# constantinpape/torch-em

Hardware: AMD Instinct MI355X
Metric: voxels/sec fwd+bwd, UNet3d 1x128^3 bs=2 (higher is better)
Workload: dtype f32-class (forward convs on normalised activations: fp32 operands split into 2 fp16 terms = 22 mantissa bits, lo plane scaled by 2^12 with its own fp32 accumulator, 3 fp16 MFMAs per product; other forward convs 3 bf16 terms / 6 MFMAs; data-gradient convs 2 bf16 terms / 3 MFMAs (16-bit products); WEI

## Files before the change

### torch_em_amd/csrc/capi.hip

```cpp
#include "tem_common.h"
#include "conv_internal.h"
#include "tem_act.h"
#include <stdarg.h>
#include <string.h>

static thread_local char g_err[512] = "";

void tem_set_error(const char* fmt, ...) {
    va_list ap;
    va_start(ap, fmt);
    vsnprintf(g_err, sizeof(g_err), fmt, ap);
    va_end(ap);
}

extern "C" const char* tem_last_error(void) { return g_err; }

struct TemOption {
    const char* name;
    long long def;
};
static const TemOption g_opt_table[TEM_OPT_COUNT] = {
    {"wgrad_zs", 3},
    {"wgrad_zs_persist", 1},
    {"wgrad_sums", 1},
    {"wgrad_sums_min_mb", 128},
    {"fwd_persistent", -1},
    {"conv_fwd_variant", -1},
    {"conv1x1_stream", 1},
    {"fwd_ksplit_chunks", 0},
    {"wgrad_cus", 256},
    {"upsample_generic", 0},
    {"team_min_units", 0},
    {"zr_splitk", 1},
    {"zr_wide", 1},
    {"zr_tile_blocks", 1},
    {"dice_vox", 1},
    {"upsample2_ch8", 1},
    {"pool_vec8", 2},
    {"fp32_zr", 1},
};
static long long g_opt_val[TEM_OPT_COUNT];
static bool g_opt_set[TEM_OPT_COUNT];

long long tem_option(int id) {
    if (id < 0 || id >= TEM_OPT_COUNT) return 0;
    return __atomic_load_n(&g_opt_set[id], __ATOMIC_RELAXED) ? __atomic_load_n(&g_opt_val[id], __ATOMIC_RELAXED)
                                                            : g_opt_table[id].def;
}
static int opt_find(const char* name) {
    if (!name) return -1;
    for (int i = 0; i < TEM_OPT_COUNT; ++i)
        if (!strcmp(name, g_opt_table[i].name)) return i;
    return -1;
}
extern "C" int tem_set_option(const char* name, int64_t value) {
    const int id = opt_find(name);
    TEM_REQUIRE(id >= 0, "tem_set_option: unknown option '%s'", name ? name : "(null)");
    __atomic_store_n(&g_opt_val[id], (long long)value, __ATOMIC_RELAXED);
    __atomic_store_n(&g_opt_set[id], true, __ATOMIC_RELAXED);
    return TEM_OK;
}
extern "C" int tem_get_option(const char* name, int64_t* value) {
    const int id = opt_find(name);
    TEM_REQUIRE(id >= 0 && value, "tem_get_option: unknown option '%s'", name ? name : "(null)");
    *value = (int64_t)tem_option(id);
    return TEM_OK;
}
extern "C" int tem_version(void) { return 100; }

extern "C" int tem_device_cus(void) {
    int dev = 0;
    if (hipGetDevice(&dev) != hipSuccess) return TEM_ELAUNCH;
// ... 169 lines not shown
```

### torch_em_amd/csrc/conv_internal.h

```cpp
#pragma once
#include <hip/hip_runtime.h>
#include <stdint.h>
#include "../../include/tem_hip.h"
#include "tem_common.h"

struct TemConvCall {
    int stx = 0;
    int sty = 0;
    int64_t x_cs = 0, y_cs = 0;
    TemByproducts* bp = nullptr;
    const unsigned* in_amax = nullptr;
    const float* ref_coef = nullptr;
    unsigned* g_amax_out = nullptr;
    const unsigned* g_amax_in = nullptr;

    bool wants(unsigned bit) const {
        if (!bp || (bp->delivered & bit)) return false;
        return bit == TEM_BP_NORM_COEF ? bp->coef != nullptr : bit == TEM_BP_NORM_SUMS ? bp->sums_part != nullptr : bp->out_amax != nullptr;
    }
    void delivered(unsigned bit) const { if (bp) bp->delivered |= bit; }
    unsigned* take_output_amax() const {
        if (!wants(TEM_BP_OUT_AMAX)) return nullptr;
        delivered(TEM_BP_OUT_AMAX);
        return bp->out_amax;
    }
};

struct TemConvShape {
    int N, D, H, W, Cin, Cout, kd, kh, kw;
    int64_t V() const { return (int64_t)D * H * W; }
    int64_t NV() const { return (int64_t)N * D * H * W; }
    int key() const { return (kd == 3) * 4 + (kh == 3) * 2 + (kw == 3); }
};

inline bool tem_plane32_ok(const TemConvShape& sh, int64_t ld) { return (int64_t)sh.H * sh.W * 8 * 4 * ld < (1ll << 31); }
inline long long tem_team_min_units(int forced) {
    const long long minu = tem_option(TEM_OPT_TEAM_MIN_UNITS);
    return tem_option(TEM_OPT_CONV_FWD_VARIANT) == forced ? 1 : (minu > 0 ? minu : 2ll * tem_ncu());
}
struct TemPatchTiling {
    bool flat;
    int TZ, TY, TX, NR;
    int64_t per, nblk;
    int ks;
};
TemPatchTiling tem_fwd_patch_tiling(const TemConvShape& sh);
struct ZrGeom {
    int shape_ok, ok;
    int nZ, nY, nX;
    int64_t nunits;
};
struct PpGeom {
    int variant;
    int TZ, TY, TX, CT, WM;
    int nZ, nY, nX;
    int64_t nunits;
};

int tem_conv_fwd_mfma(const TemPatchTiling& t, int ks, const float* x, int64_t x_ld, const float* scale, const float* shift,
                      const float* w_packed, const float* bias, float* y, int64_t y_ld, const float* ref, int64_t ref_ld, void* ws,
                      const TemConvShape& sh, int act, hipStream_t s);

int64_t tem_conv_wgrad_mfma_ws(int N, int D, int H, int W, int Cin, int Cout, int kd, int kh, int kw);
int tem_conv_wgrad_mfma(const float* x, int64_t x_ld, const float* scale, const float* shift, const float* g,
                        int64_t g_ld, float* dw_tap_ci_co, float* db, void* ws, int64_t ws_bytes, int N, int D, int H,
                        int W, int Cin, int Cout, int kd, int kh, int kw, int sd_layout, hipStream_t s);

bool tem_conv_fwd_cin1(const TemConvCall& c, const float* x, int64_t x_ld, const float* scale, const float* shift, const float* w,
                       const float* bias, float* y, int64_t y_ld, const float* ref, int N, int D, int H, int W,
                       int Cin, int Cout, int kd, int kh, int kw, int act, float* stat, hipStream_t s);
int64_t tem_conv_fwd_cin1_stat_blocks(int D, int H, int W, int Cin, int Cout, int kd, int kh, int kw);
int64_t tem_conv_wgrad_cin1_ws(int Cout, int ntaps);
bool tem_conv_wgrad_cin1(const TemConvCall& c, const float* x, int64_t x_ld, const float* scale, const float* shift, const float* g,
                         int64_t g_ld, float* dw, float* db, void* ws, int N, int D, int H, int W, int Cin, int Cout,
                         int kd, int kh, int kw, int sd_layout, const float* gnx, int64_t gnx_ld, const float* gcoef,
                         hipStream_t s);
bool tem_conv_fwd_cout1(const TemConvCall& c, const float* x, int64_t x_ld, const float* scale, const float* shift, const float* w,
                        const float* bias, float* y, int64_t y_ld, const float* ref, int N, int D, int H, int W,
                        int Cin, int Cout, int kd, int kh, int kw, int act, hipStream_t s);
bool tem_conv1x1_proj(const TemConvCall& c, const float* x, int64_t x_ld, const float* scale, const float* w, const float* bias, float* y,
                      int64_t y_ld, const float* ref, int64_t NV, int Cin, int Cout, int act, hipStream_t s);
int64_t tem_conv1x1_proj_wgrad_ws(int Cin, int Cout);
bool tem_conv1x1_proj_wgrad(const TemConvCall& c, const float* x, int64_t x_ld, const float* scale, const float* g, int64_t g_ld, float* dw,
// ... 73 lines not shown
```

### torch_em_amd/csrc/conv_zr.hip

```cpp
#include "tem_common.h"
#include "conv_internal.h"
#include "conv_arith.h"
#include "conv_split.h"
#include "tem_act.h"
#include <type_traits>

#ifndef TEM_ZR_PRIO
#define TEM_ZR_PRIO 1
#endif
#ifndef TEM_ZR_R0
#define TEM_ZR_R0 2
#endif
#ifndef TEM_ZR_R0_16
#define TEM_ZR_R0_16 2
#endif
#ifndef TEM_ZR_R0_16S
#define TEM_ZR_R0_16S 2
#endif
#ifndef TEM_ZR_AD
#define TEM_ZR_AD 2
#endif
#ifndef TEM_ZR_ST_AUX
#define TEM_ZR_ST_AUX 2
#endif
#ifndef TEM_ZR_ST_AUX_KS
#define TEM_ZR_ST_AUX_KS 2
#endif
#ifndef TEM_ZR_X32_R0_M0
#define TEM_ZR_X32_R0_M0 6
#define TEM_ZR_X32_R0_M1 4
#define TEM_ZR_X32_R0_M2 6
#define TEM_ZR_X32_R0_M3 5
#endif
#ifndef TEM_ZR_KS_FILL
#define TEM_ZR_KS_FILL 4
#endif
#ifndef TEM_ZR_ABL
#define TEM_ZR_ABL 0
#endif
#ifdef TEM_ZR_TRACE
#ifndef TEM_ZR_TRACE_BLOCK
#define TEM_ZR_TRACE_BLOCK 0
#endif
__device__ unsigned long long tem_zr_trace_buf[2][64][12];
// ... 65 lines not shown
    float a = r, b = r;
    asm volatile("s_nop 1\n\tv_permlane16_swap_b32 %0, %1" : "+v"(a), "+v"(b));
    return a + b;
}
__device__ __forceinline__ float zr_xor32_sum(float r) {
    float a = r, b = r;
    asm volatile("s_nop 1\n\tv_permlane32_swap_b32 %0, %1" : "+v"(a), "+v"(b));
    return a + b;
}

template <int CTRL>
__device__ __forceinline__ float zr_dpp(float v) {
    return __builtin_bit_cast(float, __builtin_amdgcn_update_dpp(0, __builtin_bit_cast(int, v), CTRL, 0xf, 0xf, true));
}

__device__ __forceinline__ unsigned zr_mix_lo(unsigned h, float g0, float g1) {
    unsigned q;
    const float c = -F16_LO_SCALE;
    asm("v_fma_mixlo_f16 %0, %1, %2, %3 op_sel_hi:[1,0,0]" : "=v"(q) : "v"(h), "s"(c), "v"(g0));
    asm("v_fma_mixhi_f16 %0, %1, %2, %3 op_sel:[1,0,0] op_sel_hi:[1,0,0]" : "+v"(q) : "v"(h), "s"(c), "v"(g1));
    return q;
}

__device__ __forceinline__ unsigned zr_ssel_ltu(unsigned a, unsigned b, unsigned t, unsigned f) {
    unsigned r;
    asm volatile("s_cmp_lt_u32 %1, %2\n\ts_cselect_b32 %0, %3, %4" : "=s"(r) : "s"(a), "s"(b), "s"(t), "s"(f) : "scc");
    return r;
}

struct ZrUnit {
    int cot, n, z0, y0, x0, ksl;
};

template <int NS, bool F16, int MODE, bool KSPLIT = false, bool WIDE = false, typename T = float, bool X32 = false, bool XS = false>
__global__ __launch_bounds__(XS ? 256 : 512, XS ? 1 : 2) void k_conv_zr(
    const T* __restrict__ x, int64_t x_ld, const float* __restrict__ scale, const float* __restrict__ shift,
    const uint4* __restrict__ wp, const float* __restrict__ bias, std::conditional_t<KSPLIT, float, T>* __restrict__ y, int64_t y_ld,
    const T* __restrict__ ref, int64_t ref_ld, int N, int D, int H, int W, int Cin, int Cout, int act, int nZ,
    int nY, int nX, float* __restrict__ stat, int nunits, const unsigned* __restrict__ in_amax, int ks, int blk,
    unsigned* __restrict__ out_amax, int64_t x_cs, int64_t y_cs) {
    static_assert(!KSPLIT || MODE == 0, "split-K units write raw partial sums");
    constexpr bool AMAX = MODE == 2 || MODE == 3;
    float amx = 0.f;
    static_assert(!WIDE || NS == 2, "the wide one-term kernel uses the two LDS planes of the two-term layout");
    static_assert(!X32 || (NS == 2 && !F16 && !WIDE && sizeof(T) == 4), "exact fp32: two LDS planes of eight fp32 channels, fp32 tensors");
    static_assert(!XS || X32, "the one-team workgroup exists for the exact-fp32 arithmetic only");
    constexpr bool T16 = sizeof(T) == 2;
    using TOut = std::conditional_t<KSPLIT, float, T>;
    constexpr bool Y16 = sizeof(TOut) == 2;
    constexpr int XB = (int)sizeof(T), YB = (int)sizeof(TOut);
    static_assert(!T16 || WIDE, "16-bit storage: 32 input channels per phase");
    constexpr int CK = WIDE ? 2 * BCK : BCK;
    constexpr int TZ = 4, TY = 16, TX = 8;
    constexpr int HZ = TZ + 2, HY = TY + 2, HX = TX + 2;
    constexpr int HV = HZ * HY * HX;
    constexpr int PLB = HV * 32;
    constexpr int NIT = HZ * 3;
    constexpr int LPV = (WIDE && !T16) ? 8 : 4;
    constexpr int SPP = (WIDE && !T16) ? 6 : 3;
    constexpr int CPL = T16 ? 8 : 4;
    constexpr int RP = NIT / SPP;
    constexpr int R0 = X32 ? (MODE == 0 ? TEM_ZR_X32_R0_M0 : MODE == 1 ? TEM_ZR_X32_R0_M1 : MODE == 2 ? TEM_ZR_X32_R0_M2 : TEM_ZR_X32_R0_M3)
                       : (WIDE && !T16) ? ((MODE == 1 || MODE == 3) ? 1 : 2)
                       : T16 ? ((MODE == 1 || MODE == 3) ? TEM_ZR_R0_16S : TEM_ZR_R0_16)
                             : (TEM_ZR_R0 < HZ ? TEM_ZR_R0 : HZ);
    constexpr int FR = NS * 64;
    constexpr bool SC = F16 && NS == 2 && !WIDE;
    constexpr int ZSTEP = HY * HX * 32;
    static_assert(HY % 2 == 0, "the record-half swizzle (row parity) is the same in every halo plane");
    extern __shared__ __attribute__((aligned(16))) unsigned char zr_lds[];

    if (SC) __builtin_amdgcn_s_setreg(1 | (23 << 6) | (0 << 11), 1);
    const int tid = threadIdx.x, lane = tid & 63;
    const int wv = __builtin_amdgcn_readfirstlane(tid >> 6);
    const int team = wv >> 2, tw = wv & 3, tl = tid & 255;
    const int kh = lane >> 5, v = lane & 31;
    const int vu = (int)((0x73261540u >> (4 * (v >> 2))) & 7u) * 4 + (v & 3);
    const int py = vu >> 3, px = vu & 7;
    unsigned char* lds = zr_lds + team * (NS * PLB);

    const int G = (XS ? 1 : 2) * gridDim.x;
    const int slot = XS ? tem_xcd_remap(blockIdx.x, gridDim.x) : tem_xcd_remap(blockIdx.x, gridDim.x) * 2 + team;
    const int ncot = Cout >> 5;
    const int nch_all = Cin / CK;
    const int nch = KSPLIT ? nch_all / ks : nch_all;
    const int my_units = slot < nunits ? (nunits - slot + G - 1) / G : 0;
    const int P = ((nunits + G - 1) / G) * nch;

    auto decode = [&](int ui) {
        int u = slot + ui * G;
        ZrUnit t;
        t.ksl = 0;
        if (KSPLIT) { t.ksl = u % ks; u /= ks; }
        t.cot = u % ncot; u /= ncot;
        const int lx = blk & 15, ly = (blk >> 4) & 15, lz = blk >> 8;
        const int b = u & ((1 << (lx + ly + lz)) - 1);
        u >>= lx + ly + lz;
        const int bx = b & ((1 << lx) - 1), by = (b >> lx) & ((1 << ly) - 1), bz = b >> (lx + ly);
        const int mX = nX >> lx, mY = nY >> ly, mZ = nZ >> lz;
        t.x0 = (((u % mX) << lx) + bx) * TX; u /= mX;
        t.y0 = (((u % mY) << ly) + by) * TY; u /= mY;
        t.z0 = (((u % mZ) << lz) + bz) * TZ; u /= mZ;
        t.n = u;
        return t;
    };

    const int c4 = tl & (LPV - 1);
    unsigned poff[SPP];
    unsigned lwj[SPP];
#pragma unroll
    for (int j = 0; j < SPP; ++j) {
        const int q = min((tl + 256 * j) / LPV, HY * HX - 1);
        const int hy = q / HX, hx = q % HX;
        poff[j] = ((unsigned)(hy * W + hx) * (unsigned)x_ld + (unsigned)(c4 * CPL)) * (unsigned)XB;
        if (T16 || X32)
            lwj[j] = (unsigned)(q * 32) + (unsigned)((((c4 & 1) ^ (hy & 1)) << 4)) + (unsigned)((c4 >> 1) * PLB);
        else
            lwj[j] = (unsigned)(q * 32) + (unsigned)(((((c4 >> 1) & 1) ^ (hy & 1)) << 4) | ((c4 & 1) << 3)) + (unsigned)((c4 >> 2) * PLB);
    }
    const unsigned ctr_off_ = ((unsigned)(W + 1) * (unsigned)x_ld + (unsigned)(c4 * CPL)) * (unsigned)XB;
    unsigned pvo[X32 ? SPP : 1];
    unsigned yxu = (1u << SPP) - 1u;
    auto unit_offsets = [&](const ZrUnit& t) {
        if constexpr (X32) {
            yxu = 0;
#pragma unroll
            for (int j = 0; j < SPP; ++j) {
                const int q = min((tl + 256 * j) / LPV, HY * HX - 1);
                const unsigned gy = (unsigned)(t.y0 - 1 + q / HX), gx = (unsigned)(t.x0 - 1 + q % HX);
                const bool ok = (gy < (unsigned)H) & (gx < (unsigned)W);
                yxu |= ok ? (1u << j) : 0u;
                pvo[X32 ? j : 0] = ok ? poff[j] : ctr_off_;
            }
        }
    };
    const bool slot2 = tl < (HY * HX * LPV - 256 * (SPP - 1));
    const unsigned ctr_off = ((unsigned)(W + 1) * (unsigned)x_ld + (unsigned)(c4 * CPL)) * (unsigned)XB;
    const unsigned plane_b = (unsigned)(H * W) * (unsigned)x_ld * (unsigned)XB;
    const int hvb = (4 * tw + py) * HX + px;
    const unsigned yoff_lane = ((unsigned)(4 * tw * W + (lane >> 3)) * (unsigned)y_ld + (unsigned)(4 * (lane & 7))) * (unsigned)YB;
    const unsigned roff_lane = ((unsigned)(4 * tw * W + (lane >> 3)) * (unsigned)ref_ld + (unsigned)(4 * (lane & 7))) * (unsigned)XB;
    const __amdgpu_buffer_rsrc_t rw = zr_rsrc(wp);
    const unsigned woff_lane = (unsigned)lane * 16u;
    const float act_floor = act == TEM_ACT_RELU ? 0.f : -__builtin_inff();
    float psc = 1.f, pinv = 1.f;
    if (in_amax) {
        const int e = (int)((*in_amax >> 23) & 0xffu);
        const int k = e == 0 ? 0 : min(max(141 - e, -100), 100);
        psc = __builtin_bit_cast(float, (unsigned)(127 + k) << 23);
        pinv = __builtin_bit_cast(float, (unsigned)(127 - k) << 23);
    }

    floatx16 acc[TZ];
    floatx16 accl[SC ? TZ : 1];
    const int tapstride = nch_all * FR;

    int ui = 0, ci = 0;
    ZrUnit cu = decode(0), eu = cu;
    unit_offsets(cu);
    bool epi_pending = false;
    float bv = (bias && my_units > 0) ? bias[cu.cot * 32 + v] : 0.f;
    float bve = 0.f;
    auto bias16 = [&](float* b16, float bsrc) {
#pragma unroll
        for (int i = 0; i < 16; ++i) {
            const int c0 = 8 * (i >> 2) + (i & 3);
            const float lo = __builtin_bit_cast(float, __builtin_amdgcn_readlane(__builtin_bit_cast(int, bsrc), c0));
            const float hi = __builtin_bit_cast(float, __builtin_amdgcn_readlane(__builtin_bit_cast(int, bsrc), c0 + 4));
            b16[i] = kh ? hi : lo;
        }
    };
#pragma unroll
    for (int z = 0; z < TZ; ++z)
#pragma unroll
        for (int i = 0; i < 16; ++i) {
            acc[z][i] = 0.f;
            if (SC) accl[SC ? z : 0][i] = 0.f;
        }
    unsigned wsoff = 0;

    auto epilogue_now = [&](unsigned yoff_l, unsigned roff_l, int s) {
        (void)s;
        if constexpr (X32) {
            int lane_ = (int)(threadIdx.x & 63);
            asm volatile("" : "+v"(lane_));
            const int lane = lane_, kh = lane >> 5, v = lane & 31;
            const int vu = (int)((0x73261540u >> (4 * (v >> 2))) & 7u) * 4 + (v & 3);
            const int py = vu >> 3, px = vu & 7;
            (void)py; (void)px; (void)kh;
#include "conv_zr_epilogue.inc"
        }
// ... 120 lines not shown
#pragma unroll
                    for (int pp = 0; pp < 2; ++pp) wqn[tz][pp] = zr_load4u(rw, woff_lane, wsoff_n + (unsigned)((tz * 9) * ts + pp * 64) * 16u);
                }
                stage_conv(u, tnxt);
#pragma unroll
                for (int c = 0; c < 4; ++c)
#pragma unroll
                    for (int tz = 0; tz < 3; ++tz)
#pragma unroll
                        for (int z = 0; z < TZ; ++z)
                            acc[z] = __builtin_amdgcn_mfma_f32_32x32x2f32(comp(wq[g & 1][tz][p], c), comp(xr[u & 1][z + tz], c), acc[z], 0, 0, 0);
                __builtin_amdgcn_sched_barrier(0);
            }
            if (last_chunk) {
                eu = cu;
                bve = bv;
                unsigned yo = yoff_lane, ro = roff_lane;
                asm volatile("" : "+v"(yo), "+v"(ro));
                epilogue_now(yo, ro, ph);
                bv = bias ? bias[tu.cot * 32 + v] : 0.f;
                ++ui;
            }
            cu = tu;
            ci = tc;
#pragma unroll
            for (int tz = 0; tz < 3; ++tz)
#pragma unroll
                for (int p = 0; p < 2; ++p) wq[0][tz][p] = wqn[tz][p];
            __syncthreads();
        }
        if (AMAX && out_amax) tem_amax_commit(out_amax, amx);
        return;
    }
    if (team) __syncthreads();
    for (int s = 0; s <= P; ++s) {
        const bool do_stage = ui < my_units;
        uint4 wq[2][3][NS];
        {
            ZR_STAMP(0);
#pragma unroll
            for (int j = 0; j < SPP; ++j) asm volatile("" : "+v"(lwj[j]), "+v"(poff[j]));
            unsigned yoff_l = yoff_lane, roff_l = roff_lane;
            asm volatile("" : "+v"(yoff_l), "+v"(roff_l));
            float4 tmp[NIT];
            unsigned inb[2] = {0xffffffffu, 0xffffffffu};
            float4 sc4 = make_float4(1.f, 1.f, 1.f, 1.f), sf4 = make_float4(0.f, 0.f, 0.f, 0.f);
            float4 sc5 = sc4, sf5 = sf4;
            bool interior = true;
            __amdgpu_buffer_rsrc_t rx = zr_rsrc(x);
            auto load_norm = [&]() {
                if (scale) {
                    sc4 = *reinterpret_cast<const float4*>(scale + (int64_t)cu.n * Cin + (cu.ksl * nch + ci) * CK + c4 * CPL);
                    sf4 = *reinterpret_cast<const float4*>(shift + (int64_t)cu.n * Cin + (cu.ksl * nch + ci) * CK + c4 * CPL);
                    if (T16) {
                        sc5 = *reinterpret_cast<const float4*>(scale + (int64_t)cu.n * Cin + (cu.ksl * nch + ci) * CK + c4 * CPL + 4);
                        sf5 = *reinterpret_cast<const float4*>(shift + (int64_t)cu.n * Cin + (cu.ksl * nch + ci) * CK + c4 * CPL + 4);
                    }
                } else if (in_amax) {
                    sc4 = make_float4(psc, psc, psc, psc);
                }
            };
            if (do_stage) {
                if constexpr (!X32) load_norm();
                const int64_t xch = (T16 && x_cs) ? (int64_t)(cu.ksl * nch + ci) * x_cs : (int64_t)((cu.ksl * nch + ci) * CK);
                const T* xb = x + ((((int64_t)cu.n * D + (cu.z0 - 1)) * H + (cu.y0 - 1)) * W + (cu.x0 - 1)) * x_ld + xch;
                rx = zr_rsrc((TEM_ZR_ABL & 64) ? x + xch : xb);
                interior = (cu.z0 >= 1) & (cu.z0 + HZ - 1 <= D) & (cu.y0 >= 1) & (cu.y0 + HY - 1 <= H) & (cu.x0 >= 1) &
                           (cu.x0 + HX - 1 <= W);
                if (TEM_ZR_ABL & 32) interior = true;
                if constexpr (X32) {
#pragma unroll
                    for (int hz = 0; hz < R0; ++hz) {
                        const unsigned so = zr_ssel_ltu((unsigned)(cu.z0 - 1 + hz), (unsigned)D, (unsigned)hz * plane_b, plane_b);
#pragma unroll
                        for (int j = 0; j < SPP; ++j) {
                            if (TEM_ZR_ABL & 1) tmp[hz * SPP + j] = make_float4(0.5f + hz, 0.25f, -1.f, 2.f);
                            else tmp[hz * SPP + j] = zr_load4(rx, pvo[X32 ? j : 0], so);
                        }
                    }
                    load_norm();
                }
            }
            unsigned yx = (1u << SPP) - 1u;
            if constexpr (X32) {
                if (do_stage) {
                    yx = yxu;
                    if (!interior) {
                        inb[0] = inb[1] = 0;
#pragma unroll
                        for (int hz = 0; hz < HZ; ++hz) {
                            const bool zok = (unsigned)(cu.z0 - 1 + hz) < (unsigned)D;
#pragma unroll
                            for (int j = 0; j < SPP; ++j)
                                inb[hz / 3] |= (zok & ((yx >> j) & 1u)) ? (1u << ((hz % 3) * SPP + j)) : 0u;
                        }
                    }
                }
            } else
            if (do_stage && !interior) {
                int tl_ = tl;
                asm volatile("" : "+v"(tl_));
                yx = 0;
#pragma unroll
                for (int j = 0; j < SPP; ++j) {
                    const int q = min((tl_ + 256 * j) / LPV, HY * HX - 1);
                    const unsigned gy = (unsigned)(cu.y0 - 1 + q / HX), gx = (unsigned)(cu.x0 - 1 + q % HX);
                    yx |= ((gy < (unsigned)H) & (gx < (unsigned)W)) ? (1u << j) : 0u;
                }
            }
            auto issue_loads = [&](auto interior_tag, auto lo_tag, auto hi_tag) {
                constexpr bool INTERIOR = decltype(interior_tag)::value;
                constexpr int LO = decltype(lo_tag)::value, HI = decltype(hi_tag)::value;
                if (INTERIOR) {
#pragma unroll
                    for (int hz = LO; hz < HI; ++hz)
#pragma unroll
                        for (int j = 0; j < SPP; ++j) {
                            if (TEM_ZR_ABL & 1) tmp[(hz % RP) * SPP + j] = make_float4(0.5f + hz, 0.25f, -1.f, 2.f);
                            else tmp[(hz % RP) * SPP + j] = zr_load4(rx, poff[j], (unsigned)hz * plane_b);
                        }
                } else {
                    if (LO == 0) inb[0] = inb[1] = 0;
#pragma unroll
                    for (int hz = LO; hz < HI; ++hz) {
                        const bool zok = (unsigned)(cu.z0 - 1 + hz) < (unsigned)D;
#pragma unroll
                        for (int j = 0; j < SPP; ++j) {
                            const bool ok = zok & ((yx >> j) & 1u);
                            inb[hz / 3] |= ok ? (1u << ((hz % 3) * SPP + j)) : 0u;
                            tmp[(hz % RP) * SPP + j] = zr_load4(rx, (ok ? poff[j] : ctr_off) + (ok ? (unsigned)hz * plane_b : plane_b), 0);
                        }
                    }
                }
            };
            if (do_stage && !X32) {
                if (interior) issue_loads(std::true_type{}, std::integral_constant<int, 0>{}, std::integral_constant<int, R0>{});
                else issue_loads(std::false_type{}, std::integral_constant<int, 0>{}, std::integral_constant<int, R0>{});
            }
            ZR_STAMP(1);
            if (!X32 && epi_pending) {
#include "conv_zr_epilogue.inc"
                epi_pending = false;
                ZR_STAMP(11);
            }
            ZR_STAMP(6);
            if (do_stage) {
                auto convert = [&](auto interior_tag, auto hz_tag) {
                    constexpr bool INTERIOR = decltype(interior_tag)::value;
                    constexpr int hz = decltype(hz_tag)::value;
#pragma unroll
                    for (int j = 0; j < SPP; ++j) {
                        const int it = (hz % RP) * SPP + j;
                        if constexpr (T16) {
                            if (j < SPP - 1 || slot2) {
                                u32x4z raw = __builtin_bit_cast(u32x4z, floatx4z{tmp[it].x, tmp[it].y, tmp[it].z, tmp[it].w});
                                if (scale) {
                                    raw.x = zr_norm2<F16>(raw.x, sc4.x, sf4.x, sc4.y, sf4.y);
                                    raw.y = zr_norm2<F16>(raw.y, sc4.z, sf4.z, sc4.w, sf4.w);
                                    raw.z = zr_norm2<F16>(raw.z, sc5.x, sf5.x, sc5.y, sf5.y);
                                    raw.w = zr_norm2<F16>(raw.w, sc5.z, sf5.z, sc5.w, sf5.w);
                                }
                                if (!INTERIOR) {
                                    const bool ok = ((inb[hz / 3] >> ((hz % 3) * SPP + j)) & 1u) != 0;
                                    raw.x = ok ? raw.x : 0u; raw.y = ok ? raw.y : 0u; raw.z = ok ? raw.z : 0u; raw.w = ok ? raw.w : 0u;
                                }
                                if (!(TEM_ZR_ABL & 8) || raw.x == 0x12345678u)
                                    *reinterpret_cast<uint4*>(lds + lwj[j] + hz * ZSTEP) = make_uint4(raw.x, raw.y, raw.z, raw.w);
                            }
                        } else
                        if (j < SPP - 1 || slot2) {
                            float m = 1.f;
                            if (!INTERIOR) m = ((inb[hz / 3] >> ((hz % 3) * SPP + j)) & 1u) ? 1.f : 0.f;
                            float e[4] = {fmaf(tmp[it].x, sc4.x, sf4.x), fmaf(tmp[it].y, sc4.y, sf4.y),
                                          fmaf(tmp[it].z, sc4.z, sf4.z), fmaf(tmp[it].w, sc4.w, sf4.w)};
                            if (!INTERIOR) {
#pragma unroll
                                for (int c = 0; c < 4; ++c) e[c] *= m;
                            }
                            unsigned char* dstp = lds + lwj[j] + hz * ZSTEP;
                            if constexpr (X32) {
                                if (!(TEM_ZR_ABL & 8) || e[0] == 12345.678f) *reinterpret_cast<float4*>(dstp) = make_float4(e[0], e[1], e[2], e[3]);
                            } else
                            if (SC) {
                                const half2_t hh0 = {(_Float16)e[0], (_Float16)e[1]}, hh1 = {(_Float16)e[2], (_Float16)e[3]};
                                unsigned u0 = __builtin_bit_cast(unsigned, hh0), u1 = __builtin_bit_cast(unsigned, hh1);
                                if (!(TEM_ZR_ABL & 8) || u0 == 0x12345678u) *reinterpret_cast<uint2*>(dstp) = make_uint2(u0, u1);
                                const float g[4] = {e[0] * F16_LO_SCALE, e[1] * F16_LO_SCALE, e[2] * F16_LO_SCALE, e[3] * F16_LO_SCALE};
                                const unsigned q0 = zr_mix_lo(u0, g[0], g[1]), q1 = zr_mix_lo(u1, g[2], g[3]);
                                if (!(TEM_ZR_ABL & 8) || u0 == 0x12345678u) *reinterpret_cast<uint2*>(dstp + PLB) = make_uint2(q0, q1);
                            } else if (WIDE) {
#pragma unroll
                                for (int c = 0; c < 4; ++c) asm volatile("" : "+v"(e[c]));
                                const unsigned h0 = pk16<F16>(e[0], e[1]), h1 = pk16<F16>(e[2], e[3]);
                                if (!(TEM_ZR_ABL & 8) || h0 == 0x12345678u) *reinterpret_cast<uint2*>(dstp) = make_uint2(h0, h1);
                            } else {
                                if (F16 && NS == 1) {
#pragma unroll
                                    for (int c = 0; c < 4; ++c) asm volatile("" : "+v"(e[c]));
                                }
#pragma unroll
                                for (int p = 0; p < NS; ++p) {
                                    const unsigned h0 = pk16<F16>(e[0], e[1]), h1 = pk16<F16>(e[2], e[3]);
                                    if (!(TEM_ZR_ABL & 8) || h0 == 0x12345678u)
                                        *reinterpret_cast<uint2*>(dstp + p * PLB) = make_uint2(h0, h1);
                                    if (p + 1 < NS) {
                                        e[0] -= lo16<F16>(h0);
                                        e[1] -= hi16<F16>(h0);
                                        e[2] -= lo16<F16>(h1);
                                        e[3] -= hi16<F16>(h1);
                                    }
                                }
                            }
                        }
                    }
                };
                auto stage_planes = [&](auto interior_tag) {
#define ZR_PLANE(HZI)                                                                                              \
    do {                                                                                                           \
        if ((HZI) + R0 < HZ)                                                                                       \
            issue_loads(interior_tag, std::integral_constant<int, ((HZI) + R0 < HZ ? (HZI) + R0 : 0)>{},           \
                        std::integral_constant<int, ((HZI) + R0 < HZ ? (HZI) + R0 + 1 : 0)>{});                    \
        convert(interior_tag, std::integral_constant<int, (HZI)>{});                                               \
    } while (0)
                    ZR_PLANE(0); ZR_PLANE(1); ZR_PLANE(2); ZR_PLANE(3); ZR_PLANE(4); ZR_PLANE(5);
#undef ZR_PLANE
                };
                if (interior) stage_planes(std::true_type{});
                else stage_planes(std::false_type{});
                ZR_STAMP(7);
                wsoff = (unsigned)((cu.cot * 27 * nch_all + cu.ksl * nch + ci) * FR) * 16u;
#pragma unroll
                for (int tz = 0; tz < 3; ++tz)
#pragma unroll
                    for (int p = 0; p < NS; ++p)
                        wq[0][tz][p] = zr_load4u(rw, woff_lane, wsoff + (unsigned)((tz * 9) * tapstride + p * 64) * 16u);
            }
            ZR_STAMP(2);
        }
        __syncthreads();
        {
            ZR_STAMP(3);
            if (do_stage) {
                int ts = tapstride;
                asm volatile("" : "+s"(ts));
                if (TEM_ZR_PRIO) __builtin_amdgcn_s_setprio(TEM_ZR_PRIO);
                constexpr int NSTEP = 9 * HZ;
                constexpr int AD = TEM_ZR_AD;
                uint4 af[AD + 1][NS];
                unsigned a0 = 0u;
                const unsigned hsel = (unsigned)((py & 1) ^ kh) << 4;
                int hvb_ = hvb;
                asm volatile("" : "+v"(hvb_));
                auto col_addr = [&](int g) {
                    const int hvv = hvb_ + (g / 3) * HX + (g % 3);
                    a0 = (unsigned)hvv * 32u + (((g / 3) & 1) ? hsel ^ 16u : hsel);
                };
                auto a_read = [&](int st) {
                    const int hz = st % HZ;
#pragma unroll
                    for (int p = 0; p < NS; ++p)
                        af[st % (AD + 1)][p] = *reinterpret_cast<const uint4*>(lds + a0 + hz * ZSTEP + p * PLB);
                };
                if constexpr (X32) {
                    uint4 xr[2][HZ];
                    auto r_read = [&](int u) {
                        if ((u & 1) == 0) col_addr(u >> 1);
#pragma unroll
                        for (int hz = 0; hz < HZ; ++hz)
                            xr[u & 1][hz] = *reinterpret_cast<const uint4*>(lds + a0 + hz * ZSTEP + (u & 1) * PLB);
                    };
                    auto comp = [](const uint4& q, int c) {
                        return __builtin_bit_cast(float, c == 0 ? q.x : (c == 1 ? q.y : (c == 2 ? q.z : q.w)));
                    };
                    r_read(0);
#pragma unroll
// ... 45 lines not shown
#pragma unroll
                        for (int p = 0; p < 2; ++p)
#pragma unroll
                            for (int tz = 0; tz < 3; ++tz) {
                                const int z = hz - tz;
                                if (z < 0 || z >= TZ) continue;
                                acc[z] = mfma16<F16>(wq[g & 1][tz][p], a[p], acc[z]);
                            }
                    } else
#pragma unroll
                    for (int sum = NS - 1; sum >= 0; --sum)
#pragma unroll
                        for (int i = 0; i <= sum; ++i)
#pragma unroll
                            for (int tz = 0; tz < 3; ++tz) {
                                const int z = hz - tz;
                                if (z < 0 || z >= TZ) continue;
                                if (TEM_ZR_ABL & 16) {
                                    asm volatile("" ::"v"(a[sum - i].x), "v"(a[sum - i].w), "v"(wq[g & 1][tz][i].x), "v"(wq[g & 1][tz][i].w));
                                    continue;
                                }
                                if (SC && sum == 1)
                                    accl[SC ? z : 0] = mfma16<F16>(wq[g & 1][tz][i], a[sum - i], accl[SC ? z : 0]);
                                else
                                    acc[z] = mfma16<F16>(wq[g & 1][tz][i], a[sum - i], acc[z]);
                            }
                    __builtin_amdgcn_sched_barrier(0);
                }
                }
                if (TEM_ZR_PRIO) __builtin_amdgcn_s_setprio(0);
            }
            ZR_STAMP(4);
        }
        if (do_stage) {
            if (++ci == nch) {
                ci = 0;
                eu = cu;
                epi_pending = !X32;
                bve = bv;
                if constexpr (X32) {
                    unsigned yo = yoff_lane, ro = roff_lane;
                    asm volatile("" : "+v"(yo), "+v"(ro));
                    epilogue_now(yo, ro, s);
                }
                bv = 0.f;
                if (++ui < my_units) {
                    cu = decode(ui);
                    if (bias) bv = bias[cu.cot * 32 + v];
                    unit_offsets(cu);
                }
            }
        }
        __syncthreads();
        ZR_STAMP(5);
    }
    if (!team) __syncthreads();
    if (AMAX && out_amax) tem_amax_commit(out_amax, amx);
}

ZrGeom tem_zr_geometry(const TemConvCall& c, const TemConvShape& sh, int mode) {
    ZrGeom g = {};
    const long long opt = tem_option(TEM_OPT_CONV_FWD_VARIANT);
    if (opt == 0 || opt == 1) return g;
    if (!tem_zr_takes(mode, c, sh.Cin)) return g;
    if (sh.key() != 7 || sh.D < 4 || sh.Cin % 16 || sh.Cout % 32) return g;
    g.shape_ok = 1;
    g.nZ = (sh.D + 3) / 4;
    g.nY = (sh.H + 15) / 16;
    g.nX = (sh.W + 7) / 8;
    g.nunits = (int64_t)sh.N * g.nZ * g.nY * g.nX * (sh.Cout / 32);
    g.ok = g.nunits < (1ll << 31) && g.nunits >= tem_team_min_units(2);
    return g;
}

static int zr_tile_blocks(const ZrGeom& g) {
    if (!tem_option(TEM_OPT_ZR_TILE_BLOCKS)) return 0;
    auto lg = [](int n) { return n % 4 == 0 ? 2 : (n % 2 == 0 ? 1 : 0); };
    return lg(g.nX) | (lg(g.nY) << 4) | (lg(g.nZ) << 8);
}

template <int NS, bool F16, int MODE, bool KSPLIT = false, bool WIDE = false, typename T = float, bool X32 = false, bool XS = false>
static void zr_launch(const TemConvCall& c, const ZrGeom& g, const float* x_, int64_t x_ld, const float* scale, const float* shift, const float* wp,
                      const float* bias, float* y_, int64_t y_ld, const float* ref_, int64_t ref_ld, const TemConvShape& sh,
                      int act, float* stat, const unsigned* in_amax, hipStream_t s, int ks = 1) {
    constexpr size_t ldsb = (size_t)2 * NS * 1080 * 32 + 4 * 32 * 144;
    static_assert(ldsb <= 160 * 1024, "LDS budget");
    const T* x = reinterpret_cast<const T*>(x_);
    const T* ref = reinterpret_cast<const T*>(ref_);
    auto* y = reinterpret_cast<std::conditional_t<KSPLIT, float, T>*>(y_);
    auto kern = &k_conv_zr<NS, F16, MODE, KSPLIT, WIDE, T, X32, XS>;
    static bool attr = false;
    if (!attr) {
        (void)hipFuncSetAttribute(reinterpret_cast<const void*>(kern), hipFuncAttributeMaxDynamicSharedMemorySize, (int)ldsb);
        attr = true;
    }
    const int64_t nunits = g.nunits * ks;
    int64_t grid = XS ? nunits : (nunits + 1) / 2;
    if (grid > tem_ncu()) grid = tem_ncu();
    unsigned* const out_amax = (MODE == 2 || MODE == 3) ? c.take_output_amax() : nullptr;
    hipLaunchKernelGGL(kern, dim3((unsigned)grid), dim3(XS ? 256 : 512), ldsb, s, x, x_ld, scale, shift, reinterpret_cast<const uint4*>(wp),
                       bias, y, y_ld, ref, ref_ld, sh.N, sh.D, sh.H, sh.W, sh.Cin, sh.Cout, act, g.nZ, g.nY, g.nX, stat, (int)nunits, in_amax, ks,
                       zr_tile_blocks(g), out_amax, (int64_t)(sizeof(T) == 2 ? c.x_cs : 0), (int64_t)(sizeof(T) == 2 && !KSPLIT ? c.y_cs : 0));
}

template <int NS_, bool F16_, bool WIDE_ = false, typename T_ = float, bool X32_ = false, bool XS_ = false>
struct ZrVariant {
    static constexpr int NS = NS_;
    static constexpr bool F16 = F16_, WIDE = WIDE_, X32 = X32_, XS = XS_;
    using T = T_;
};
template <typename F>
static void zr_variant(const TemConvCall& c, int mode, bool wide, F&& f) {
    const TemArith& a = tem_arith(mode);
    if (c.stx == TEM_ST_F16) f(ZrVariant<2, true, true, tem_f16>{});
    else if (c.stx == TEM_ST_BF16) f(ZrVariant<2, false, true, tem_bf16>{});
    else if (mode == TEM_ARITH_FP32 && tem_option(TEM_OPT_FP32_ZR) == 2) f(ZrVariant<2, false, false, float, true, true>{});
    else if (mode == TEM_ARITH_FP32) f(ZrVariant<2, false, false, float, true>{});
    else if (a.planes == 1 && wide) tem_select_bool(a.elem == TEM_EL_F16, [&](auto f16) { f(ZrVariant<2, f16(), true>{}); });
    else if (a.planes == 1) tem_select_bool(a.elem == TEM_EL_F16, [&](auto f16) { f(ZrVariant<1, f16()>{}); });
    else tem_select_bool(a.pack == TEM_PK_F16_LO12, [&](auto f16) { f(ZrVariant<2, f16()>{}); });
}

int tem_zr_splitk_ks(const TemConvCall& c, const ZrGeom& g, const TemConvShape& sh, int mode) {
// ... 55 lines not shown
```

### torch_em_amd/csrc/tem_common.h

```cpp
#pragma once
#include <hip/hip_runtime.h>
#include <stdint.h>
#include <stdio.h>
#include "../../include/tem_hip.h"

void tem_set_error(const char* fmt, ...);

enum {
    TEM_OPT_WGRAD_ZS = 0,
    TEM_OPT_WGRAD_ZS_PERSIST,
    TEM_OPT_WGRAD_SUMS,
    TEM_OPT_WGRAD_SUMS_MIN_MB,
    TEM_OPT_FWD_PERSISTENT,
    TEM_OPT_CONV_FWD_VARIANT,
    TEM_OPT_CONV1X1_STREAM,
    TEM_OPT_FWD_KSPLIT_CHUNKS,
    TEM_OPT_WGRAD_CUS,
    TEM_OPT_UPSAMPLE_GENERIC,
    TEM_OPT_TEAM_MIN_UNITS,
    TEM_OPT_ZR_SPLITK,
    TEM_OPT_ZR_WIDE,
    TEM_OPT_ZR_TILE_BLOCKS,
    TEM_OPT_DICE_VOX,
    TEM_OPT_UPSAMPLE2_CH8,
    TEM_OPT_POOL_VEC8,
    TEM_OPT_FP32_ZR,
    TEM_OPT_COUNT
};
long long tem_option(int id);
int tem_ncu();

#define TEM_REQUIRE(cond, ...)                 \
    do {                                       \
        if (!(cond)) {                         \
            tem_set_error(__VA_ARGS__);        \
            return TEM_EINVAL;                 \
        }                                      \
    } while (0)

#define TEM_TRY(call)                          \
    do {                                       \
        const int rc__ = (call);               \
        if (rc__ != TEM_OK) return rc__;       \
    } while (0)

#define TEM_CHECK_LAUNCH(name)                                                   \
    do {                                                                         \
        hipError_t e__ = hipGetLastError();                                      \
        if (e__ != hipSuccess) {                                                 \
            tem_set_error("%s: launch failed: %s", name, hipGetErrorString(e__)); \
            return TEM_ELAUNCH;                                                  \
        }                                                                        \
    } while (0)

static inline int64_t tem_cdiv(int64_t a, int64_t b) { return (a + b - 1) / b; }
static inline int64_t tem_align_up(int64_t a, int64_t b) { return tem_cdiv(a, b) * b; }

static inline int tem_grid_1d(int64_t work_items, int block, int max_blocks = 256 * 8) {
    int64_t g = tem_cdiv(work_items, block);
// ... 37 lines not shown
```

Before: 275.6 million.

## Pair sibling teams to co-stage halves of one halo tile in shared LDS buffers

Adds a PAIR variant of the zero-redundancy forward conv kernel. The two teams in a workgroup each stage half of the z-halo planes of the same tile into a shared, double-buffered LDS region, and one team lags a step behind so that staging and MFMA tap work overlap. Unit decode is reordered so sibling slots share an input tile across output-channel tiles, and the pipeline runs one extra iteration with a conditional barrier. The aim is to halve per-team global loads and LDS staging. In exchange the sibling teams are now coupled, which adds synchronisation and some complexity in the barrier logic. It is enabled by default for fp32 two-plane modes when Cout is a multiple of 64.

```diff
diff --git a/torch_em_amd/csrc/capi.hip b/torch_em_amd/csrc/capi.hip
--- a/torch_em_amd/csrc/capi.hip
+++ b/torch_em_amd/csrc/capi.hip
@@ -38,6 +38,7 @@
     {"upsample2_ch8", 1},
     {"pool_vec8", 2},
     {"fp32_zr", 1},
+    {"zr_pair", 1},
 };
 static long long g_opt_val[TEM_OPT_COUNT];
 static bool g_opt_set[TEM_OPT_COUNT];
diff --git a/torch_em_amd/csrc/conv_internal.h b/torch_em_amd/csrc/conv_internal.h
--- a/torch_em_amd/csrc/conv_internal.h
+++ b/torch_em_amd/csrc/conv_internal.h
@@ -49,6 +49,7 @@
     int shape_ok, ok;
     int nZ, nY, nX;
     int64_t nunits;
+    int pair;
 };
 struct PpGeom {
     int variant;
diff --git a/torch_em_amd/csrc/conv_zr.hip b/torch_em_amd/csrc/conv_zr.hip
--- a/torch_em_amd/csrc/conv_zr.hip
+++ b/torch_em_amd/csrc/conv_zr.hip
@@ -10,6 +10,9 @@
 #endif
 #ifndef TEM_ZR_R0
 #define TEM_ZR_R0 2
+#endif
+#ifndef TEM_ZR_R0_PAIR
+#define TEM_ZR_R0_PAIR 1
 #endif
 #ifndef TEM_ZR_R0_16
 #define TEM_ZR_R0_16 2
@@ -141,7 +144,7 @@
     int cot, n, z0, y0, x0, ksl;
 };
 
-template <int NS, bool F16, int MODE, bool KSPLIT = false, bool WIDE = false, typename T = float, bool X32 = false, bool XS = false>
+template <int NS, bool F16, int MODE, bool KSPLIT = false, bool WIDE = false, typename T = float, bool X32 = false, bool XS = false, bool PAIR = false>
 __global__ __launch_bounds__(XS ? 256 : 512, XS ? 1 : 2) void k_conv_zr(
     const T* __restrict__ x, int64_t x_ld, const float* __restrict__ scale, const float* __restrict__ shift,
     const uint4* __restrict__ wp, const float* __restrict__ bias, std::conditional_t<KSPLIT, float, T>* __restrict__ y, int64_t y_ld,
@@ -154,6 +157,7 @@
     static_assert(!WIDE || NS == 2, "the wide one-term kernel uses the two LDS planes of the two-term layout");
     static_assert(!X32 || (NS == 2 && !F16 && !WIDE && sizeof(T) == 4), "exact fp32: two LDS planes of eight fp32 channels, fp32 tensors");
     static_assert(!XS || X32, "the one-team workgroup exists for the exact-fp32 arithmetic only");
+    static_assert(!PAIR || (NS == 2 && !WIDE && !X32 && sizeof(T) == 4), "sibling pairing: the two-term split modes on fp32 tensors");
     constexpr bool T16 = sizeof(T) == 2;
     using TOut = std::conditional_t<KSPLIT, float, T>;
     constexpr bool Y16 = sizeof(TOut) == 2;
@@ -164,7 +168,9 @@
     constexpr int HZ = TZ + 2, HY = TY + 2, HX = TX + 2;
     constexpr int HV = HZ * HY * HX;
     constexpr int PLB = HV * 32;
-    constexpr int NIT = HZ * 3;
+    constexpr bool HALF = PAIR || ((TEM_ZR_ABL & 128) && !X32 && !WIDE && !T16);
+    constexpr int HZS = HALF ? HZ / 2 : HZ;
+    constexpr int NIT = HZS * 3;
     constexpr int LPV = (WIDE && !T16) ? 8 : 4;
     constexpr int SPP = (WIDE && !T16) ? 6 : 3;
     constexpr int CPL = T16 ? 8 : 4;
@@ -172,7 +178,9 @@
     constexpr int R0 = X32 ? (MODE == 0 ? TEM_ZR_X32_R0_M0 : MODE == 1 ? TEM_ZR_X32_R0_M1 : MODE == 2 ? TEM_ZR_X32_R0_M2 : TEM_ZR_X32_R0_M3)
                        : (WIDE && !T16) ? ((MODE == 1 || MODE == 3) ? 1 : 2)
                        : T16 ? ((MODE == 1 || MODE == 3) ? TEM_ZR_R0_16S : TEM_ZR_R0_16)
+                       : HALF ? TEM_ZR_R0_PAIR
                              : (TEM_ZR_R0 < HZ ? TEM_ZR_R0 : HZ);
+    static_assert(R0 >= 1 && R0 <= HZS, "planes requested ahead: at least one, at most what the team stages");
     constexpr int FR = NS * 64;
     constexpr bool SC = F16 && NS == 2 && !WIDE;
     constexpr int ZSTEP = HY * HX * 32;
@@ -186,7 +194,7 @@
     const int kh = lane >> 5, v = lane & 31;
     const int vu = (int)((0x73261540u >> (4 * (v >> 2))) & 7u) * 4 + (v & 3);
     const int py = vu >> 3, px = vu & 7;
-    unsigned char* lds = zr_lds + team * (NS * PLB);
+    const int hzb = HALF ? (HZ / 2) * team : 0;
 
     const int G = (XS ? 1 : 2) * gridDim.x;
     const int slot = XS ? tem_xcd_remap(blockIdx.x, gridDim.x) : tem_xcd_remap(blockIdx.x, gridDim.x) * 2 + team;
@@ -200,8 +208,9 @@
         int u = slot + ui * G;
         ZrUnit t;
         t.ksl = 0;
-        if (KSPLIT) { t.ksl = u % ks; u /= ks; }
+        if (KSPLIT && !PAIR) { t.ksl = u % ks; u /= ks; }
         t.cot = u % ncot; u /= ncot;
+        if (KSPLIT && PAIR) { t.ksl = u % ks; u /= ks; }
         const int lx = blk & 15, ly = (blk >> 4) & 15, lz = blk >> 8;
         const int b = u & ((1 << (lx + ly + lz)) - 1);
         u >>= lx + ly + lz;
@@ -266,6 +275,9 @@
 
     int ui = 0, ci = 0;
     ZrUnit cu = decode(0), eu = cu;
+    ZrUnit su = cu;
+    int sui = 0, sci = 0;
+    const int lag = (PAIR && team == 0) ? 1 : 0;
     unit_offsets(cu);
     bool epi_pending = false;
     float bv = (bias && my_units > 0) ? bias[cu.cot * 32 + v] : 0.f;
@@ -452,9 +464,14 @@
         if (AMAX && out_amax) tem_amax_commit(out_amax, amx);
         return;
     }
-    if (team) __syncthreads();
-    for (int s = 0; s <= P; ++s) {
-        const bool do_stage = ui < my_units;
+    if (team && !PAIR) __syncthreads();
+    for (int s = 0; s <= P + (PAIR ? 1 : 0); ++s) {
+        const bool do_tap = s >= lag && ui < my_units;
+        const bool do_stage = PAIR ? sui < my_units : do_tap;
+        const ZrUnit& stu = PAIR ? su : cu;
+        const int stc = PAIR ? sci : ci;
+        unsigned char* const slds = zr_lds + (PAIR ? (s & 1) : team) * (NS * PLB) + hzb * ZSTEP;
+        const unsigned char* const lds = zr_lds + (PAIR ? ((s - lag) & 1) : team) * (NS * PLB);
         uint4 wq[2][3][NS];
         {
             ZR_STAMP(0);
@@ -470,11 +487,11 @@
             __amdgpu_buffer_rsrc_t rx = zr_rsrc(x);
             auto load_norm = [&]() {
                 if (scale) {
-                    sc4 = *reinterpret_cast<const float4*>(scale + (int64_t)cu.n * Cin + (cu.ksl * nch + ci) * CK + c4 * CPL);
-                    sf4 = *reinterpret_cast<const float4*>(shift + (int64_t)cu.n * Cin + (cu.ksl * nch + ci) * CK + c4 * CPL);
+                    sc4 = *reinterpret_cast<const float4*>(scale + (int64_t)stu.n * Cin + (stu.ksl * nch + stc) * CK + c4 * CPL);
+                    sf4 = *reinterpret_cast<const float4*>(shift + (int64_t)stu.n * Cin + (stu.ksl * nch + stc) * CK + c4 * CPL);
                     if (T16) {
-                        sc5 = *reinterpret_cast<const float4*>(scale + (int64_t)cu.n * Cin + (cu.ksl * nch + ci) * CK + c4 * CPL + 4);
-                        sf5 = *reinterpret_cast<const float4*>(shift + (int64_t)cu.n * Cin + (cu.ksl * nch + ci) * CK + c4 * CPL + 4);
+                        sc5 = *reinterpret_cast<const float4*>(scale + (int64_t)stu.n * Cin + (stu.ksl * nch + stc) * CK + c4 * CPL + 4);
+                        sf5 = *reinterpret_cast<const float4*>(shift + (int64_t)stu.n * Cin + (stu.ksl * nch + stc) * CK + c4 * CPL + 4);
                     }
                 } else if (in_amax) {
                     sc4 = make_float4(psc, psc, psc, psc);
@@ -482,11 +499,11 @@
             };
             if (do_stage) {
                 if constexpr (!X32) load_norm();
-                const int64_t xch = (T16 && x_cs) ? (int64_t)(cu.ksl * nch + ci) * x_cs : (int64_t)((cu.ksl * nch + ci) * CK);
-                const T* xb = x + ((((int64_t)cu.n * D + (cu.z0 - 1)) * H + (cu.y0 - 1)) * W + (cu.x0 - 1)) * x_ld + xch;
+                const int64_t xch = (T16 && x_cs) ? (int64_t)(stu.ksl * nch + stc) * x_cs : (int64_t)((stu.ksl * nch + stc) * CK);
+                const T* xb = x + ((((int64_t)stu.n * D + (stu.z0 - 1)) * H + (stu.y0 - 1)) * W + (stu.x0 - 1)) * x_ld + xch;
                 rx = zr_rsrc((TEM_ZR_ABL & 64) ? x + xch : xb);
-                interior = (cu.z0 >= 1) & (cu.z0 + HZ - 1 <= D) & (cu.y0 >= 1) & (cu.y0 + HY - 1 <= H) & (cu.x0 >= 1) &
-                           (cu.x0 + HX - 1 <= W);
+                interior = (stu.z0 >= 1) & (stu.z0 + HZ - 1 <= D) & (stu.y0 >= 1) & (stu.y0 + HY - 1 <= H) & (stu.x0 >= 1) &
+                           (stu.x0 + HX - 1 <= W);
                 if (TEM_ZR_ABL & 32) interior = true;
                 if constexpr (X32) {
 #pragma unroll
@@ -524,7 +541,7 @@
 #pragma unroll
                 for (int j = 0; j < SPP; ++j) {
                     const int q = min((tl_ + 256 * j) / LPV, HY * HX - 1);
-                    const unsigned gy = (unsigned)(cu.y0 - 1 + q / HX), gx = (unsigned)(cu.x0 - 1 + q % HX);
+                    const unsigned gy = (unsigned)(stu.y0 - 1 + q / HX), gx = (unsigned)(stu.x0 - 1 + q % HX);
                     yx |= ((gy < (unsigned)H) & (gx < (unsigned)W)) ? (1u << j) : 0u;
                 }
             }
@@ -537,18 +554,18 @@
 #pragma unroll
                         for (int j = 0; j < SPP; ++j) {
                             if (TEM_ZR_ABL & 1) tmp[(hz % RP) * SPP + j] = make_float4(0.5f + hz, 0.25f, -1.f, 2.f);
-                            else tmp[(hz % RP) * SPP + j] = zr_load4(rx, poff[j], (unsigned)hz * plane_b);
+                            else tmp[(hz % RP) * SPP + j] = zr_load4(rx, poff[j], (unsigned)(hzb + hz) * plane_b);
                         }
                 } else {
                     if (LO == 0) inb[0] = inb[1] = 0;
 #pragma unroll
                     for (int hz = LO; hz < HI; ++hz) {
-                        const bool zok = (unsigned)(cu.z0 - 1 + hz) < (unsigned)D;
+                        const bool zok = (unsigned)(stu.z0 - 1 + hzb + hz) < (unsigned)D;
 #pragma unroll
                         for (int j = 0; j < SPP; ++j) {
                             const bool ok = zok & ((yx >> j) & 1u);
                             inb[hz / 3] |= ok ? (1u << ((hz % 3) * SPP + j)) : 0u;
-                            tmp[(hz % RP) * SPP + j] = zr_load4(rx, (ok ? poff[j] : ctr_off) + (ok ? (unsigned)hz * plane_b : plane_b), 0);
+                            tmp[(hz % RP) * SPP + j] = zr_load4(rx, (ok ? poff[j] : ctr_off) + (ok ? (unsigned)(hzb + hz) * plane_b : plane_b), 0);
                         }
                     }
                 }
@@ -585,7 +602,7 @@
                                     raw.x = ok ? raw.x : 0u; raw.y = ok ? raw.y : 0u; raw.z = ok ? raw.z : 0u; raw.w = ok ? raw.w : 0u;
                                 }
                                 if (!(TEM_ZR_ABL & 8) || raw.x == 0x12345678u)
-                                    *reinterpret_cast<uint4*>(lds + lwj[j] + hz * ZSTEP) = make_uint4(raw.x, raw.y, raw.z, raw.w);
+                                    *reinterpret_cast<uint4*>(slds + lwj[j] + hz * ZSTEP) = make_uint4(raw.x, raw.y, raw.z, raw.w);
                             }
                         } else
                         if (j < SPP - 1 || slot2) {
@@ -597,7 +614,7 @@
 #pragma unroll
                                 for (int c = 0; c < 4; ++c) e[c] *= m;
                             }
-                            unsigned char* dstp = lds + lwj[j] + hz * ZSTEP;
+                            unsigned char* dstp = slds + lwj[j] + hz * ZSTEP;
                             if constexpr (X32) {
                                 if (!(TEM_ZR_ABL & 8) || e[0] == 12345.678f) *reinterpret_cast<float4*>(dstp) = make_float4(e[0], e[1], e[2], e[3]);
                             } else
@@ -637,17 +654,20 @@
                 auto stage_planes = [&](auto interior_tag) {
 #define ZR_PLANE(HZI)                                                                                              \
     do {                                                                                                           \
-        if ((HZI) + R0 < HZ)                                                                                       \
-            issue_loads(interior_tag, std::integral_constant<int, ((HZI) + R0 < HZ ? (HZI) + R0 : 0)>{},           \
-                        std::integral_constant<int, ((HZI) + R0 < HZ ? (HZI) + R0 + 1 : 0)>{});                    \
+        if ((HZI) + R0 < HZS)                                                                                      \
+            issue_loads(interior_tag, std::integral_constant<int, ((HZI) + R0 < HZS ? (HZI) + R0 : 0)>{},          \
+                        std::integral_constant<int, ((HZI) + R0 < HZS ? (HZI) + R0 + 1 : 0)>{});                   \
         convert(interior_tag, std::integral_constant<int, (HZI)>{});                                               \
     } while (0)
-                    ZR_PLANE(0); ZR_PLANE(1); ZR_PLANE(2); ZR_PLANE(3); ZR_PLANE(4); ZR_PLANE(5);
+                    ZR_PLANE(0); ZR_PLANE(1); ZR_PLANE(2);
+                    if constexpr (HZS == HZ) { ZR_PLANE(3); ZR_PLANE(4); ZR_PLANE(5); }
 #undef ZR_PLANE
                 };
                 if (interior) stage_planes(std::true_type{});
                 else stage_planes(std::false_type{});
                 ZR_STAMP(7);
+            }
+            if (do_tap) {
                 wsoff = (unsigned)((cu.cot * 27 * nch_all + cu.ksl * nch + ci) * FR) * 16u;
 #pragma unroll
                 for (int tz = 0; tz < 3; ++tz)
@@ -660,7 +680,7 @@
         __syncthreads();
         {
             ZR_STAMP(3);
-            if (do_stage) {
+            if (do_tap) {
                 int ts = tapstride;
                 asm volatile("" : "+s"(ts));
                 if (TEM_ZR_PRIO) __builtin_amdgcn_s_setprio(TEM_ZR_PRIO);
@@ -772,7 +792,13 @@
             }
             ZR_STAMP(4);
         }
-        if (do_stage) {
+        if (PAIR && do_stage) {
+            if (++sci == nch) {
+                sci = 0;
+                if (++sui < my_units) su = decode(sui);
+            }
+        }
+        if (do_tap) {
             if (++ci == nch) {
                 ci = 0;
                 eu = cu;
@@ -791,7 +817,7 @@
                 }
             }
         }
-        __syncthreads();
+        if (!(PAIR && lag && s == 0)) __syncthreads();
         ZR_STAMP(5);
     }
     if (!team) __syncthreads();
@@ -810,6 +836,7 @@
     g.nX = (sh.W + 7) / 8;
     g.nunits = (int64_t)sh.N * g.nZ * g.nY * g.nX * (sh.Cout / 32);
     g.ok = g.nunits < (1ll << 31) && g.nunits >= tem_team_min_units(2);
+    g.pair = tem_option(TEM_OPT_ZR_PAIR) && sh.Cout % 64 == 0 && c.stx == TEM_ST_F32 && mode != TEM_ARITH_FP32 && tem_arith(mode).planes == 2;
     return g;
 }
 
@@ -819,7 +846,7 @@
     return lg(g.nX) | (lg(g.nY) << 4) | (lg(g.nZ) << 8);
 }
 
-template <int NS, bool F16, int MODE, bool KSPLIT = false, bool WIDE = false, typename T = float, bool X32 = false, bool XS = false>
+template <int NS, bool F16, int MODE, bool KSPLIT = false, bool WIDE = false, typename T = float, bool X32 = false, bool XS = false, bool PAIR = false>
 static void zr_launch(const TemConvCall& c, const ZrGeom& g, const float* x_, int64_t x_ld, const float* scale, const float* shift, const float* wp,
                       const float* bias, float* y_, int64_t y_ld, const float* ref_, int64_t ref_ld, const TemConvShape& sh,
                       int act, float* stat, const unsigned* in_amax, hipStream_t s, int ks = 1) {
@@ -828,7 +855,10 @@
     const T* x = reinterpret_cast<const T*>(x_);
     const T* ref = reinterpret_cast<const T*>(ref_);
     auto* y = reinterpret_cast<std::conditional_t<KSPLIT, float, T>*>(y_);
-    auto kern = &k_conv_zr<NS, F16, MODE, KSPLIT, WIDE, T, X32, XS>;
+    if constexpr (!PAIR && NS == 2 && !WIDE && !X32 && sizeof(T) == 4) {
+        if (g.pair) return zr_launch<NS, F16, MODE, KSPLIT, WIDE, T, X32, XS, true>(c, g, x_, x_ld, scale, shift, wp, bias, y_, y_ld, ref_, ref_ld, sh, act, stat, in_amax, s, ks);
+    }
+    auto kern = &k_conv_zr<NS, F16, MODE, KSPLIT, WIDE, T, X32, XS, PAIR>;
     static bool attr = false;
     if (!attr) {
         (void)hipFuncSetAttribute(reinterpret_cast<const void*>(kern), hipFuncAttributeMaxDynamicSharedMemorySize, (int)ldsb);
diff --git a/torch_em_amd/csrc/tem_common.h b/torch_em_amd/csrc/tem_common.h
--- a/torch_em_amd/csrc/tem_common.h
+++ b/torch_em_amd/csrc/tem_common.h
@@ -25,6 +25,7 @@
     TEM_OPT_UPSAMPLE2_CH8,
     TEM_OPT_POOL_VEC8,
     TEM_OPT_FP32_ZR,
+    TEM_OPT_ZR_PAIR,
     TEM_OPT_COUNT
 };
 long long tem_option(int id);
```

After: 278.5 million, median of 6. +1.1%, better.
